# openjamoses/TOSEM-2021-Replication

Measured on NVIDIA H100. Metric: source MB/s scanned (tokenise + line-hash + classify + aggregate), higher is better.
Workload: dtype u8

## Files before the change

tosem-2021-replication_b200/csrc/tsm_scan_walk.cuh:

```cuda
#pragma once
#include "tsm_scan_kernels.cuh"

namespace tsm {

#ifndef TSM_SCAN2_WARPS
#define TSM_SCAN2_WARPS 11
#endif
#ifndef TSM_SCAN2_CTAS
#define TSM_SCAN2_CTAS 2
#endif
#ifndef TSM_WALK_UNROLL
#define TSM_WALK_UNROLL 1
#endif
constexpr int SCAN2_WARPS = TSM_SCAN2_WARPS, SCAN2_CTAS_PER_SM = TSM_SCAN2_CTAS, WALK_UNROLL = TSM_WALK_UNROLL;

constexpr uint32_t NWORD = BUF / 8;
constexpr uint32_t O2_ARUN = BUF;
constexpr uint32_t SLOT_TAIL = NWORD;
constexpr uint32_t RW2_PER_STRIPE = 4;
constexpr uint32_t O2_RW = O2_ARUN + ((NWORD + 1) * 4 + 7) / 8 * 8;
constexpr uint32_t O2_WENT = O2_RW + 32 * RW2_PER_STRIPE * 8;
constexpr uint32_t WENT_CAP = NWORD + 8;
constexpr uint32_t LCAP = 512;
constexpr uint32_t O2_LTAB = O2_WENT + WENT_CAP * 2;
constexpr uint32_t O2_BASE = O2_LTAB + (LCAP + 8) * 2;
constexpr uint32_t Q2_CAP = 64;
constexpr uint32_t O2_Q = O2_BASE + 34 * 8;
constexpr uint32_t O2_CTL = O2_Q + Q2_CAP * 2;
constexpr uint32_t WARP_SMEM2 = ((O2_CTL + 16 + 127) / 128) * 128;
#ifndef TSM_PHASE_CLOCKS
#define TSM_PHASE_CLOCKS 0
#endif
enum ScanPhase { PH_WAIT, PH_ZERO, PH_WALK, PH_SCANS, PH_MIXED, PH_RECORDS, PH_FINISH, PH_LONG, PH_FLUSH, PH_N };
#if TSM_PHASE_CLOCKS
__device__ unsigned long long g_scan_phase_clk[PH_N];
#endif
struct PhaseClock {
#if TSM_PHASE_CLOCKS
  uint32_t* tab;
  long long t;
  __device__ __forceinline__ void mark(int ph, int lane) {
    const long long now = clock64();
    if (lane == 0) atomicAdd(tab + ph, (uint32_t)(now - t));
    t = now;
  }
#else
  __device__ __forceinline__ void mark(int, int) {}
#endif
};

constexpr uint32_t O2_T0A = LUT_BYTES;
constexpr uint32_t O2_PHASE = LUT_BYTES + 512;
constexpr uint32_t CTA_BYTES2 = LUT_BYTES + 512 + (TSM_PHASE_CLOCKS ? 128 : 0);
constexpr uint32_t SCAN2_SMEM = CTA_BYTES2 + SCAN2_WARPS * WARP_SMEM2;
constexpr uint32_t O2_LUTB = SCAN2_SMEM;
constexpr uint32_t SCAN2_SMEM_B = SCAN2_SMEM + 1024;
static_assert(O2_RW % 8 == 0 && O2_WENT % 8 == 0 && O2_LTAB % 2 == 0 && O2_BASE % 8 == 0 && O2_Q % 4 == 0 && O2_CTL % 8 == 0, "alignment");
static_assert(SCAN2_CTAS_PER_SM * (SCAN2_SMEM_B + 1024) <= 233472, "shared memory per SM (228 KB, 1 KB reserved per CTA)");
constexpr uint32_t LR_POS = 0x1FFFu, LR_FIRST = 0x2000u, LR_MIXED = 0x4000u, LR_VIRT = 0x8000u;

constexpr uint32_t B2_FIRST = (1u << 0) | (1u << 6) | (1u << 15), B2_FIN = (1u << 5) | (1u << 14) | (1u << 18);
constexpr uint32_t REVB_BIT = 1u;

struct LutRef { uint32_t four, base; };
__device__ __forceinline__ LutRef lut_ref() { return LutRef{scan_lut()[256 + 12], scan_lut()[256 + 13]}; }
template <bool REVB>
__device__ __forceinline__ void lut_at(uint32_t idx, LutRef t, uint32_t& v, uint32_t& v2) {
  uint32_t addr;
  asm("mad.lo.u32 %0, %1, %2, %3;" : "=r"(addr) : "r"(idx), "r"(t.four), "r"(t.base));
  asm("ld.shared.u32 %0, [%1];" : "=r"(v) : "r"(addr));
  if (REVB) asm("ld.shared.u32 %0, [%1+%2];" : "=r"(v2) : "r"(addr), "n"(O2_LUTB));
}

struct Auto { uint32_t D, D2; };

template <bool REVB>
__device__ __forceinline__ uint32_t step1(Auto& a, uint32_t byte, LutRef t) {
  uint32_t m, m2 = 0;
  lut_at<REVB>(byte, t, m, m2);
  a.D = ((a.D + a.D) | B_FIRST) & m;
  if (!REVB) return a.D;
  a.D2 = ((a.D2 + a.D2) | B2_FIRST) & m2;
  return (a.D & ~REVB_BIT) | ((a.D2 & B2_FIN) ? REVB_BIT : 0u);
}

template <bool REVB>
__device__ __forceinline__ void step8b(unsigned long long w, Auto& a, uint32_t& A, LutRef t) {
  const uint32_t lo = (uint32_t)w, hi = (uint32_t)(w >> 32);
  uint32_t A2 = 0;
#pragma unroll
  for (int k = 0; k < 8; ++k) {
    uint32_t m, m2 = 0;
    lut_at<REVB>(__byte_perm(k < 4 ? lo : hi, 0, 0x4440 + (k & 3)), t, m, m2);
    a.D = ((a.D + a.D) | B_FIRST) & m;
    A |= a.D;
    if (REVB) { a.D2 = ((a.D2 + a.D2) | B2_FIRST) & m2; A2 |= a.D2; }
  }
  if (REVB) A = (A & ~REVB_BIT) | ((A2 & B2_FIN) ? REVB_BIT : 0u);
}

__device__ __forceinline__ uint32_t nl8_of(unsigned long long w) {
  return nl_word((uint32_t)w) | (nl_word((uint32_t)(w >> 32)) << 4);
}
__device__ __forceinline__ unsigned long long low_mask(uint32_t b) {
  return b >= 8u ? ~0ull : ((1ull << (8u * b)) - 1ull);
}
__device__ __forceinline__ unsigned long long ror3_61(unsigned long long r) { return (r >> 3) + ((r & 7ull) << 58); }

struct WalkOut { uint32_t nlw, tail; };

template <bool REVB>
__device__ __noinline__ WalkOut walk2(uint8_t* wb, uint32_t fin, int lane) {
  const uint32_t pos0 = (uint32_t)lane * STRIPE;
  const uint8_t* sp = wb + pos0;
  uint32_t* ar = reinterpret_cast<uint32_t*>(wb + O2_ARUN) + (uint32_t)lane * 17u;
  unsigned long long* rw = reinterpret_cast<unsigned long long*>(wb + O2_RW) + (uint32_t)lane * RW2_PER_STRIPE;
  const LutRef t = lut_ref();
  Auto au{0u, 0u};
  if (lane) {
    uint32_t A = 0;
    step8b<REVB>(*reinterpret_cast<const unsigned long long*>(sp - 8), au, A, t);
  }
  unsigned long long R = 0;
  uint32_t run = 0, nlr = 0;
  auto word = [&](uint32_t k) {
    const unsigned long long w = *reinterpret_cast<const unsigned long long*>(sp + 8u * k);
    uint32_t A = 0;
    step8b<REVB>(w, au, A, t);
    R = ror3_61(R) + fold61(w);
    ar[k] = run;
    nlr = __funnelshift_l(A, nlr, 1);
    const bool nl = (int32_t)A < 0;
    if (nl && (A & fin)) {
      const uint32_t slot = atomicAdd(reinterpret_cast<uint32_t*>(wb + O2_CTL), 1u);
      if (slot < Q2_CAP) reinterpret_cast<uint16_t*>(wb + O2_Q)[slot] = (uint16_t)((uint32_t)lane * 17u + k);
    }
    run = nl ? 0u : (run | A);
  };
#pragma unroll 1
  for (uint32_t g = 0; g < 4; ++g) {
#pragma unroll WALK_UNROLL
    for (uint32_t k = 0; k < 4; ++k) word(4u * g + k);
    rw[g] = R;
  }
  word(16);
  unsigned long long incl = rotl61(canon61(R), (3u * (17u * (uint32_t)lane + 16u)) % 61u);
#pragma unroll
  for (int d = 1; d < 32; d <<= 1) {
    const unsigned long long t = __shfl_up_sync(0xffffffffu, incl, d);
    if (lane >= d) incl = fold61(incl + t);
  }
  unsigned long long excl = __shfl_up_sync(0xffffffffu, incl, 1);
  if (lane == 0) excl = 0;
  unsigned long long* sbase = reinterpret_cast<unsigned long long*>(wb + O2_BASE);
  sbase[lane] = excl;
  if (lane == 31) sbase[32] = incl;
  return WalkOut{__brev(nlr) >> 15, run};
}

template <bool REVB>
__device__ __noinline__ void resolve_mixed(uint8_t* wb, uint32_t g, uint32_t i, uint32_t n_went) {
  const LutRef t = lut_ref();
  Auto au{0u, 0u};
  uint32_t A = 0;
  step8b<REVB>(*reinterpret_cast<const unsigned long long*>(wb + 8u * g - 8u), au, A, t);
  unsigned long long w = *reinterpret_cast<const unsigned long long*>(wb + 8u * g);
  uint32_t pre = 0, post = 0, seen = 0;
#pragma unroll
  for (int b = 0; b < 8; ++b) {
    const uint32_t d = step1<REVB>(au, (uint32_t)w & 0xFFu, t);
    const uint32_t m = (uint32_t)((int32_t)au.D >> 31);
    pre |= d & ~seen;
    seen |= m;
    post = (post | d) & ~m;
    w >>= 8;
  }
  uint32_t* arun = reinterpret_cast<uint32_t*>(wb + O2_ARUN);
  const uint16_t* went = reinterpret_cast<const uint16_t*>(wb + O2_WENT);
  atomicOr(arun + g, pre);
  const uint32_t tgt = i + 1u < n_went ? ((uint32_t)went[i + 1u] & 0x3FFu) : SLOT_TAIL;
  atomicOr(arun + tgt, post);
}

__device__ __forceinline__ void emit_header(const ScanParams& p, uint32_t f, uint32_t line_off, uint32_t len, uint32_t fl) {
  const uint32_t slot = atomicAdd(&p.ctrl->n_hev, 1u);
  if (slot < p.hev_cap) p.hev[slot] = tsm_header_event{f, line_off, len, (fl >> 2) & 1u};
  else p.ctrl->overflow = 1;
}

template <typename Bytes>
__device__ __noinline__ bool starts_with8(Bytes lb, uint32_t s, uint32_t e, unsigned long long pat, uint32_t n, bool need_ws) {
  uint32_t r;
  while (s + 8 <= e && (r = lb.spaces8(s)) != 0) { s += r; if (r < 8) break; }
  while (s < e && is_w(lb(s))) ++s;
  if (s + n + (need_ws ? 1u : 0u) > e) return false;
  const unsigned long long v = lb.load8(s);
  if ((v & low_mask(n)) != pat) return false;
  if (need_ws) {
    const uint32_t c = (uint32_t)(v >> (8u * n)) & 0xFFu;
    if (c != 0x20 && c != 0x09) return false;
    for (uint32_t q = s + n + 1; q < e; ++q)
      if (!is_w(lb(q))) return true;
    return false;
  }
  return true;
}

template <bool REVB, typename Bytes>
__device__ __forceinline__ uint32_t line_flags2(uint32_t s, uint32_t e, uint32_t A, uint32_t g1, uint32_t g2, int ext, Bytes lb, Accum& ac) {
  if (ext == 0) return 0;
  uint32_t fl = (A & (AF_ASSERT | AF_EXPECT | (REVB ? REVB_BIT : 0u))) ? LF_CAND : 0;
  bool hdr;
  if (ext == TSM_EXT_PY) {
    hdr = (A & g1) != 0;
    if (!hdr && (A & g2)) hdr = starts_with8(lb, s, e, 0x7373616C63ull, 5, true);
  } else {
    hdr = (A & g1) != 0 && (A & g2) != 0;
  }
  if (hdr) { fl |= LF_HDR; if ((A & B_F) && starts_with8(lb, s, e, 0x465F54534554ull, 6, false)) fl |= LF_FIX; }
  ac.asserts += fl & LF_CAND;
  ac.hdrs += (fl >> 1) & 1u;
  ac.fixes += (fl >> 2) & 1u;
  return fl;
}

struct FinishState {
  Accum ac;
  uint32_t prev_last;
  unsigned long long prevP;
  uint32_t lh_base, lh_done;
};

template <bool REVB>
__device__ __noinline__ FinishState finish_lines2(const ScanParams& p, uint8_t* wb, const uint32_t* lc, uint32_t n, uint32_t lim,
                                                  bool skip_first, uint32_t f, uint32_t cb, int ext, int lane, FinishState fs) {
  uint16_t* ltab = reinterpret_cast<uint16_t*>(wb + O2_LTAB);
  const uint32_t* arun = reinterpret_cast<const uint32_t*>(wb + O2_ARUN);
  const unsigned long long* t0a = reinterpret_cast<const unsigned long long*>(scan_lut()) + O2_T0A / 8;
  const uint32_t g1 = lc[1], g2 = lc[2];
  const SmemByte lb{wb};
  const bool want_hev = (p.flags & TSM_SCAN_HEADER_EVENTS) != 0, want_lh = (p.flags & TSM_SCAN_LINE_HASHES) != 0;
  Accum a = fs.ac;
  uint32_t nc = 0, lh_done = fs.lh_done;
  uint32_t prev_last = fs.prev_last;
  unsigned long long prevP = fs.prevP;
  for (uint32_t base = 0; base < n; base += 32) {
    const uint32_t j = base + (uint32_t)lane;
    const bool valid = j < n;
    const uint32_t rec = valid ? (uint32_t)ltab[j] : 0u;
    const uint32_t e = rec & LR_POS;
    const bool isv = (rec & LR_VIRT) != 0;
    const uint32_t g = min(e >> 3, NWORD - 1u), b1 = e - 8u * g + (isv ? 0u : 1u);
    const uint32_t l = g / 17u, i = g - 17u * l, c0 = i >> 2, ns = i & 3u;
    unsigned long long R = 0;
    if (c0) R = *reinterpret_cast<const unsigned long long*>(wb + O2_RW + 8u * (l * RW2_PER_STRIPE + c0 - 1u));
    const unsigned long long* wp = reinterpret_cast<const unsigned long long*>(wb) + (g - ns);
#pragma unroll
    for (uint32_t t = 0; t < 3u; ++t)
      if (ns > t) R = ror3_61(R) + fold61(wp[t]);
    const unsigned long long w = *reinterpret_cast<const unsigned long long*>(wb + 8u * g);
    const uint32_t r3g = (3u * g) % 61u;
    const unsigned long long X = ror3_61(R) + fold61(w & low_mask(b1));
    unsigned long long Pn = *reinterpret_cast<const unsigned long long*>(wb + O2_BASE + 8u * l) + rotl61(fold61(fold61(X)), r3g);
    uint32_t r8e = r3g + 8u * (e & 7u);
    if (r8e >= 61u) r8e -= 61u;
    const unsigned long long Pe = isv ? Pn : Pn + M61 - t0a[r8e];
    uint32_t s = __shfl_up_sync(0xffffffffu, e, 1) + 1u;
    unsigned long long Ps = __shfl_up_sync(0xffffffffu, Pn, 1);
    if (lane == 0) { s = prev_last + 1u; Ps = prevP; }
    const int src = base + 32u <= n ? 31 : (int)(n - 1u - base);
    prev_last = __shfl_sync(0xffffffffu, e, src);
    prevP = __shfl_sync(0xffffffffu, Pn, src);
    const bool owned = valid && s < lim && !(s == PRE && skip_first);
    uint32_t fl = 0;
    unsigned long long lh = 0;
    if (owned) {
      const unsigned long long hr = canon61(Pe + 4ull * M61 - Ps);
      const uint32_t sh = (8u * s) % 61u;
      unsigned long long h = rotl61(hr, sh ? 61u - sh : 0u);
      uint32_t len = e - s;
      if (len && lb(e - 1u) == 0x0D) {
        --len;
        const unsigned long long cr = rotl61(0x0Dull, (8u * len) % 61u);
        h = h >= cr ? h - cr : h + M61 - cr;
      }
      a.lines++;
      lh = mix_hash(h, len);
      a.digest += lh;
      uint32_t A = 0;
      if (rec & LR_FIRST) A = arun[isv ? SLOT_TAIL : g];
      else if (rec & LR_MIXED) {
        Auto au{0u, 0u};
        const LutRef t = lut_ref();
        for (uint32_t q = s; q < e; ++q) A |= step1<REVB>(au, lb(q), t);
      }
      fl = line_flags2<REVB>(s, e, A, g1, g2, ext, lb, a);
      if (want_hev && (fl & LF_HDR)) emit_header(p, f, cb + s - PRE, e - s, fl);
    }
    if (want_lh) {
      const uint32_t mo = __ballot_sync(0xffffffffu, owned);
      const uint32_t slot = fs.lh_base + lh_done + __popc(mo & ((1u << lane) - 1u));
      if (owned && slot < p.lh_cap) {
        p.lh_hash[slot] = lh;
        p.lh_end[slot] = cb + e - PRE;
        p.lh_flag[slot] = (uint8_t)(fl & LF_CAND);
      }
      lh_done += __popc(mo);
    }
    __syncwarp();
    const uint32_t mc = __ballot_sync(0xffffffffu, fl & LF_CAND);
    if (fl & LF_CAND) ltab[nc + __popc(mc & ((1u << lane) - 1u))] = (uint16_t)s;
    nc += __popc(mc);
  }
  __syncwarp();
  if (nc && p.cand_cap) {
    const uint32_t cbase = warp_reserve(&p.ctrl->n_cand, nc, lane);
    for (uint32_t i = (uint32_t)lane; i < nc; i += 32) {
      const uint32_t slot = cbase + i;
      if (slot < p.cand_cap) p.cand[slot] = ((unsigned long long)f << 32) | (cb + (uint32_t)ltab[i] - PRE);
      else p.ctrl->overflow = 1;
    }
  }
  __syncwarp();
  fs.ac = a;
  fs.prev_last = prev_last;
  fs.prevP = prevP;
  fs.lh_done = lh_done;
  return fs;
}

template <bool REVB>
__device__ __noinline__ Accum long_line(const ScanParams& p, const uint32_t* lc, uint32_t f, uint32_t size, int ext,
                                        uint32_t s, uint32_t lh_slot, Accum ac) {
  const HbmByte lb{p.arena + (uint32_t)p.off[f]};
  uint32_t e = s;
  while (e < size && lb(e) != '\n') ++e;
  const uint32_t k0 = s >> 3, k1 = (e - 1u) >> 3;
  const LutRef t = lut_ref();
  Auto au{0u, 0u};
  uint32_t A = 0;
  unsigned long long R = 0;
#pragma unroll 1
  for (uint32_t k = k0; k <= k1; ++k) {
    unsigned long long w = __ldg(reinterpret_cast<const unsigned long long*>(lb.b) + k);
    if (k == k0) w &= ~0ull << (8u * (s & 7u));
    if (k == k1) w &= low_mask(e - 8u * k);
    uint32_t Aw = 0;
    step8b<REVB>(w, au, Aw, t);
    A |= Aw;
    R = ror3_61(R) + fold61(w);
  }
  unsigned long long h = rotl61(canon61(R), (3u * (k1 - k0) + 61u * 8u - 8u * (s & 7u)) % 61u);
  uint32_t len = e - s;
  if (lb(e - 1u) == 0x0D) {
    --len;
    const unsigned long long cr = rotl61(0x0Dull, (8u * len) % 61u);
    h = h >= cr ? h - cr : h + M61 - cr;
  }
  const unsigned long long lh = mix_hash(h, len);
  ac.lines++;
  ac.digest += lh;
  const uint32_t fl = line_flags2<REVB>(s, e, A, lc[1], lc[2], ext, lb, ac);
  if ((fl & LF_CAND) && p.cand_cap) {
    const uint32_t slot = atomicAdd(&p.ctrl->n_cand, 1u);
    if (slot < p.cand_cap) p.cand[slot] = ((unsigned long long)f << 32) | s;
    else p.ctrl->overflow = 1;
  }
  if ((fl & LF_HDR) && (p.flags & TSM_SCAN_HEADER_EVENTS)) emit_header(p, f, s, e - s, fl);
  if ((p.flags & TSM_SCAN_LINE_HASHES) && lh_slot < p.lh_cap) {
    p.lh_hash[lh_slot] = lh;
    p.lh_end[lh_slot] = e;
    p.lh_flag[lh_slot] = (uint8_t)(fl & LF_CAND);
  }
  return ac;
}

template <bool REVB>
__device__ __forceinline__ void process_chunk2(const ScanParams& p, const uint32_t* lc, uint8_t* wb, uint32_t uslot, uint32_t f,
                                               uint32_t cb, uint32_t size, int ext, int lane, PhaseClock& pc) {
  const uint32_t ce = min(cb + CH, size);
  const uint32_t le = min(ce + EXT, size);
  const uint32_t lim = PRE + (ce - cb);
  const uint32_t lim2 = PRE + (le - cb);
  const bool skip_first = (cb != 0) && (wb[PRE - 1] != '\n');
  __syncwarp();
  if (lane < 2) reinterpret_cast<unsigned long long*>(wb)[lane] = 0ull;
  {
    const uint32_t za = (lim2 + 7u) & ~7u;
    if ((uint32_t)lane < za - lim2) wb[lim2 + lane] = 0;
    for (uint32_t q = za + 8u * (uint32_t)lane; q < BUF; q += 256u) *reinterpret_cast<unsigned long long*>(wb + q) = 0ull;
  }
  if (lane == 0) *reinterpret_cast<uint32_t*>(wb + O2_CTL) = 0u;
  __syncwarp();
  pc.mark(PH_ZERO, lane);
  const WalkOut wo = walk2<REVB>(wb, lc[0], lane);
  pc.mark(PH_WALK, lane);
  const uint32_t w0 = 17u * (uint32_t)lane, lim_w = (lim + 7u) >> 3;
  const uint32_t ownbits = lim_w <= w0 ? 0u : (lim_w - w0 >= 17u ? 0x1FFFFu : (1u << (lim_w - w0)) - 1u);
  const uint32_t extbits = wo.nlw & ~ownbits;
  const uint32_t gx = __reduce_min_sync(0xffffffffu, extbits ? w0 + (uint32_t)__ffs((int)extbits) - 1u : 0xFFFFu);
  uint32_t kept = wo.nlw & ownbits;
  if (gx - w0 < 17u) kept |= 1u << (gx - w0);
  uint32_t tv = wo.tail, tf = wo.nlw != 0u;
  const uint32_t cnt = __popc(kept);
  uint32_t incl = cnt;
#pragma unroll
  for (int d = 1; d < 32; d <<= 1) {
    const uint32_t uv = __shfl_up_sync(0xffffffffu, tv, d), uf = __shfl_up_sync(0xffffffffu, tf, d);
    const uint32_t t = __shfl_up_sync(0xffffffffu, incl, d);
    if (lane >= d) { if (!tf) tv |= uv; tf |= uf; incl += t; }
  }
  uint32_t carry = __shfl_up_sync(0xffffffffu, tv, 1);
  if (lane == 0) carry = 0;
  const uint32_t tail_all = __shfl_sync(0xffffffffu, tv, 31);
  const uint32_t n_went = __shfl_sync(0xffffffffu, incl, 31), ebase = incl - cnt;
  uint16_t* went = reinterpret_cast<uint16_t*>(wb + O2_WENT);
  uint32_t* arun = reinterpret_cast<uint32_t*>(wb + O2_ARUN);
  {
    uint32_t b = kept, idx = ebase;
    while (b) { went[idx++] = (uint16_t)(w0 + (uint32_t)__ffs((int)b) - 1u); b &= b - 1u; }
    if (wo.nlw) arun[w0 + (uint32_t)__ffs((int)wo.nlw) - 1u] |= carry;
    if (lane == 0) arun[SLOT_TAIL] = tail_all;
  }
  __syncwarp();
  pc.mark(PH_SCANS, lane);
  {
    const uint32_t nq_all = *reinterpret_cast<const uint32_t*>(wb + O2_CTL);
    const uint16_t* q = reinterpret_cast<const uint16_t*>(wb + O2_Q);
    if (nq_all <= Q2_CAP) {
      for (uint32_t base = 0; base < nq_all; base += 32) {
        const uint32_t t = base + (uint32_t)lane;
        const uint32_t g = t < nq_all ? (uint32_t)q[t] : 0u;
        const uint32_t l = g / 17u, k = g - 17u * l;
        const uint32_t m = __shfl_sync(0xffffffffu, kept, (int)l), eb = __shfl_sync(0xffffffffu, ebase, (int)l);
        const bool act = t < nq_all && ((m >> k) & 1u);
        const uint32_t i = eb + __popc(m & ((1u << k) - 1u));
        if (act) resolve_mixed<REVB>(wb, g, i, n_went);
        __syncwarp();
        if (act) went[i] |= 0x8000u;
        __syncwarp();
      }
    } else if (lc[0]) {
      for (uint32_t base = 0; base < n_went; base += 32) {
        const uint32_t i = base + (uint32_t)lane;
        if (i < n_went) resolve_mixed<REVB>(wb, (uint32_t)went[i] & 0x3FFu, i, n_went);
        __syncwarp();
        if (i < n_went) went[i] |= 0x8000u;
        __syncwarp();
      }
    }
  }
  pc.mark(PH_MIXED, lane);
  uint16_t* ltab = reinterpret_cast<uint16_t*>(wb + O2_LTAB);
  FinishState fs{{0, 0, 0, 0, 0}, PRE - 1u, 0ull, 0u, 0u};
  const bool want_lh = (p.flags & TSM_SCAN_LINE_HASHES) != 0;
  if (want_lh) {
    uint32_t tot = 0;
    for (uint32_t j = (uint32_t)lane; j < n_went; j += 32)
      tot += __popc(nl8_of(*reinterpret_cast<const unsigned long long*>(wb + 8u * ((uint32_t)went[j] & 0x3FFu))));
    tot = __reduce_add_sync(0xffffffffu, tot) + 1u;
    uint32_t base = 0;
    if (lane == 0) {
      base = atomicAdd(&p.ctrl->n_lh, tot);
      if (base + tot > p.lh_cap) p.ctrl->lh_overflow = 1;
      p.unit_out[uslot] = base;
    }
    fs.lh_base = __shfl_sync(0xffffffffu, base, 0);
  }
  uint32_t n_rec = 0, last_nl = PRE - 1u;
  for (uint32_t base = 0; base < n_went; base += 32) {
    const uint32_t j = base + (uint32_t)lane;
    const uint32_t ge = j < n_went ? (uint32_t)went[j] : 0u;
    const uint32_t g = ge & 0x3FFu;
    uint32_t m = j < n_went ? nl8_of(*reinterpret_cast<const unsigned long long*>(wb + 8u * g)) : 0u;
    const uint32_t c = __popc(m);
    uint32_t in2 = c;
#pragma unroll
    for (int d = 1; d < 32; d <<= 1) {
      const uint32_t t = __shfl_up_sync(0xffffffffu, in2, d);
      if (lane >= d) in2 += t;
    }
    if (base + 32u >= n_went) {
      const uint32_t lastl = n_went - 1u - base;
      last_nl = __shfl_sync(0xffffffffu, 8u * g + 31u - (uint32_t)__clz((int)(m | 1u)), (int)lastl);
    }
    uint32_t off = n_rec + in2 - c;
    uint32_t rec = 8u * g + LR_FIRST + ((ge >> 15) << 14);
    while (m) {
      ltab[off++] = (uint16_t)(rec + (uint32_t)__ffs((int)m) - 1u);
      rec &= ~LR_FIRST;
      m &= m - 1u;
    }
    n_rec += __shfl_sync(0xffffffffu, in2, 31);
    __syncwarp();
    if (n_rec + 256u > LCAP && base + 32u < n_went) {
      pc.mark(PH_RECORDS, lane);
      fs = finish_lines2<REVB>(p, wb, lc, n_rec, lim, skip_first, f, cb, ext, lane, fs);
      pc.mark(PH_FINISH, lane);
      n_rec = 0;
    }
  }
  const uint32_t tail_start = last_nl + 1u;
  bool tail_long = false;
  if (tail_start < lim && !(skip_first && n_went == 0u)) {
    if (le == size) {
      if (tail_start < lim2) { if (lane == 0) ltab[n_rec] = (uint16_t)(lim2 | LR_VIRT | LR_FIRST); ++n_rec; }
    } else tail_long = true;
  }
  __syncwarp();
  pc.mark(PH_RECORDS, lane);
  if (n_rec) fs = finish_lines2<REVB>(p, wb, lc, n_rec, lim, skip_first, f, cb, ext, lane, fs);
  pc.mark(PH_FINISH, lane);
  Accum ac = fs.ac;
  if (tail_long && lane == 0) ac = long_line<REVB>(p, lc, f, size, ext, cb + tail_start - PRE, fs.lh_base + fs.lh_done, ac);
  pc.mark(PH_LONG, lane);
  ac.lines = __reduce_add_sync(0xffffffffu, ac.lines);
  ac.asserts = __reduce_add_sync(0xffffffffu, ac.asserts);
  ac.hdrs = __reduce_add_sync(0xffffffffu, ac.hdrs);
  ac.fixes = __reduce_add_sync(0xffffffffu, ac.fixes);
  {
    const uint32_t dlo = (uint32_t)ac.digest, dhi = (uint32_t)(ac.digest >> 32);
    const unsigned long long s0 = __reduce_add_sync(0xffffffffu, dlo & 0xFFFFu);
    const unsigned long long s1 = __reduce_add_sync(0xffffffffu, dlo >> 16);
    const unsigned long long s2 = __reduce_add_sync(0xffffffffu, dhi);
    ac.digest = s0 + (s1 << 16) + (s2 << 32);
  }
  if (want_lh && lane == 0) p.unit_lines[uslot] = ac.lines;
  if (lane == 0) {
    tsm_file_stat* st = p.stats + f;
    if (size <= CH) {
      *st = tsm_file_stat{ac.lines, ac.asserts, ac.hdrs, ac.fixes, ac.digest};
    } else {
      if (ac.lines) atomicAdd(&st->n_lines, ac.lines);
      if (ac.asserts) atomicAdd(&st->n_assert, ac.asserts);
      if (ac.hdrs) atomicAdd(&st->n_headers, ac.hdrs);
      if (ac.fixes) atomicAdd(&st->n_fixture, ac.fixes);
      if (ac.digest) atomicAdd(reinterpret_cast<unsigned long long*>(&st->digest), ac.digest);
    }
  }
  pc.mark(PH_FLUSH, lane);
}

template <bool REVB>
__global__ void __launch_bounds__(SCAN2_WARPS * 32, SCAN2_CTAS_PER_SM) k_scan_t(const __grid_constant__ ScanParams p) {
  extern __shared__ __align__(128) uint8_t smem[];
  uint32_t* lut_all = reinterpret_cast<uint32_t*>(smem);
  for (int i = threadIdx.x; i < 256; i += blockDim.x) lut_all[i] = c_lut[i];
  if (threadIdx.x < 12) {
    const int t = threadIdx.x, lang = t >> 2, q = t & 3;
    const uint32_t g1 = lang == 0 ? PY_G1 : CJ_G1, g2 = lang == 0 ? PY_G2 : CJ_G2;
    const uint32_t v = q == 0 ? (AF_ASSERT | AF_EXPECT | g1 | g2 | B_F | (REVB ? REVB_BIT : 0u)) : (q == 1 ? g1 : (q == 2 ? g2 : 0u));
    lut_all[256 + t] = lang == 2 ? 0u : v;
  }
  if (threadIdx.x == 12) lut_all[256 + 12] = p.four;
  if (threadIdx.x == 13) lut_all[256 + 13] = smem_u32(lut_all);
  if (REVB) for (int i = threadIdx.x; i < 256; i += blockDim.x) lut_all[O2_LUTB / 4 + i] = c_lut_b[i];
  PhaseClock pc;
#if TSM_PHASE_CLOCKS
  pc.tab = reinterpret_cast<uint32_t*>(smem + O2_PHASE);
  if (threadIdx.x < PH_N) pc.tab[threadIdx.x] = 0u;
#endif
  if (threadIdx.x >= 32 && threadIdx.x < 32 + 61)
    reinterpret_cast<unsigned long long*>(smem + O2_T0A)[threadIdx.x - 32] = rotl61(0x0Aull, threadIdx.x - 32);
  __syncthreads();
  const int warp = threadIdx.x >> 5, lane = threadIdx.x & 31;
  uint8_t* wb = smem + CTA_BYTES2 + warp * WARP_SMEM2;
  uint64_t* bar = reinterpret_cast<uint64_t*>(wb + O2_CTL + 8);
  uint32_t* phase = reinterpret_cast<uint32_t*>(wb + O2_CTL + 4);
  if (lane == 0) { mbar_init(bar, 1); fence_mbar_init(); *phase = 0u; }
  __syncwarp();
  const uint32_t n_units = p.slab->n_units;
  Unit cur = claim_unit(p, n_units, lane);
#if TSM_PHASE_CLOCKS
  pc.t = clock64();
#endif
  while (cur.u < n_units) {
    fence_proxy_async();
    __syncwarp();
    if (lane == 0) issue_load(p, wb, bar, cur.fo, cur.size, cur.cb);
    const Unit nxt = claim_unit(p, n_units, lane);
    const uint32_t ph = *phase;
    while (!mbar_try_wait(bar, ph)) {}
    __syncwarp();
    if (lane == 0) *phase = ph ^ 1u;
    pc.mark(PH_WAIT, lane);
    const uint32_t lang = cur.ext == 0 ? 2u : (cur.ext == TSM_EXT_PY ? 0u : 1u);
    process_chunk2<REVB>(p, lut_all + 256u + 4u * lang, wb, p.unit_base + cur.u, cur.f, cur.cb, cur.size, cur.ext, lane, pc);
    __syncwarp();
    cur = nxt;
  }
#if TSM_PHASE_CLOCKS
  __syncthreads();
  if (threadIdx.x < PH_N) atomicAdd(&g_scan_phase_clk[threadIdx.x], (unsigned long long)pc.tab[threadIdx.x]);
#endif
}

template __global__ void k_scan_t<false>(const __grid_constant__ ScanParams);
template __global__ void k_scan_t<true>(const __grid_constant__ ScanParams);

}
```

Measured before the change: 616,900.

## Hash lines from end-inclusive prefix and subtract newline constant algebraically

Each line hash now uses the prefix value that includes the terminating byte at each line end (Pe) rather than a separate pre-newline prefix. A constant-shift correction for the preceding newline is subtracted after the rotation, which removes the per-CTA shared-memory rotation table and its per-line lookup. The warp shuffles are merged so the carry from the last lane comes from one indexed shuffle, the prefix-fold loop is made branch-free, and header and fix counters are incremented inside the branch. This cuts shared-memory loads and shuffles per line, but correctness depends on the modular identity holding for virtual line ends and for the initial carry value.

Result: no change. 618,500 (median of 6 runs) (+0.3%).

```diff
diff --git a/tosem-2021-replication_b200/csrc/tsm_scan_walk.cuh b/tosem-2021-replication_b200/csrc/tsm_scan_walk.cuh
--- a/tosem-2021-replication_b200/csrc/tsm_scan_walk.cuh
+++ b/tosem-2021-replication_b200/csrc/tsm_scan_walk.cuh
@@ -49,9 +49,8 @@
 #endif
 };
 
-constexpr uint32_t O2_T0A = LUT_BYTES;
-constexpr uint32_t O2_PHASE = LUT_BYTES + 512;
-constexpr uint32_t CTA_BYTES2 = LUT_BYTES + 512 + (TSM_PHASE_CLOCKS ? 128 : 0);
+constexpr uint32_t O2_PHASE = LUT_BYTES;
+constexpr uint32_t CTA_BYTES2 = LUT_BYTES + (TSM_PHASE_CLOCKS ? 128 : 0);
 constexpr uint32_t SCAN2_SMEM = CTA_BYTES2 + SCAN2_WARPS * WARP_SMEM2;
 constexpr uint32_t O2_LUTB = SCAN2_SMEM;
 constexpr uint32_t SCAN2_SMEM_B = SCAN2_SMEM + 1024;
@@ -217,17 +216,21 @@
   } else {
     hdr = (A & g1) != 0 && (A & g2) != 0;
   }
-  if (hdr) { fl |= LF_HDR; if ((A & B_F) && starts_with8(lb, s, e, 0x465F54534554ull, 6, false)) fl |= LF_FIX; }
+  if (hdr) {
+    fl |= LF_HDR;
+    ac.hdrs++;
+    if ((A & B_F) && starts_with8(lb, s, e, 0x465F54534554ull, 6, false)) { fl |= LF_FIX; ac.fixes++; }
+  }
   ac.asserts += fl & LF_CAND;
-  ac.hdrs += (fl >> 1) & 1u;
-  ac.fixes += (fl >> 2) & 1u;
   return fl;
 }
+
+constexpr unsigned long long NL_BEFORE = 0x0Aull << 53;
 
 struct FinishState {
   Accum ac;
   uint32_t prev_last;
-  unsigned long long prevP;
+  unsigned long long prevPe;
   uint32_t lh_base, lh_done;
 };
 
@@ -236,41 +239,42 @@
                                                   bool skip_first, uint32_t f, uint32_t cb, int ext, int lane, FinishState fs) {
   uint16_t* ltab = reinterpret_cast<uint16_t*>(wb + O2_LTAB);
   const uint32_t* arun = reinterpret_cast<const uint32_t*>(wb + O2_ARUN);
-  const unsigned long long* t0a = reinterpret_cast<const unsigned long long*>(scan_lut()) + O2_T0A / 8;
   const uint32_t g1 = lc[1], g2 = lc[2];
   const SmemByte lb{wb};
   const bool want_hev = (p.flags & TSM_SCAN_HEADER_EVENTS) != 0, want_lh = (p.flags & TSM_SCAN_LINE_HASHES) != 0;
   Accum a = fs.ac;
   uint32_t nc = 0, lh_done = fs.lh_done;
   uint32_t prev_last = fs.prev_last;
-  unsigned long long prevP = fs.prevP;
+  unsigned long long prevPe = fs.prevPe;
   for (uint32_t base = 0; base < n; base += 32) {
     const uint32_t j = base + (uint32_t)lane;
     const bool valid = j < n;
     const uint32_t rec = valid ? (uint32_t)ltab[j] : 0u;
     const uint32_t e = rec & LR_POS;
     const bool isv = (rec & LR_VIRT) != 0;
-    const uint32_t g = min(e >> 3, NWORD - 1u), b1 = e - 8u * g + (isv ? 0u : 1u);
+    const uint32_t g = min(e >> 3, NWORD - 1u), b1 = e - 8u * g;
     const uint32_t l = g / 17u, i = g - 17u * l, c0 = i >> 2, ns = i & 3u;
     unsigned long long R = 0;
     if (c0) R = *reinterpret_cast<const unsigned long long*>(wb + O2_RW + 8u * (l * RW2_PER_STRIPE + c0 - 1u));
     const unsigned long long* wp = reinterpret_cast<const unsigned long long*>(wb) + (g - ns);
 #pragma unroll
-    for (uint32_t t = 0; t < 3u; ++t)
-      if (ns > t) R = ror3_61(R) + fold61(wp[t]);
+    for (uint32_t t = 0; t < 3u; ++t) {
+      const unsigned long long Rt = ror3_61(R) + fold61(wp[t]);
+      R = ns > t ? Rt : R;
+    }
     const unsigned long long w = *reinterpret_cast<const unsigned long long*>(wb + 8u * g);
-    const uint32_t r3g = (3u * g) % 61u;
     const unsigned long long X = ror3_61(R) + fold61(w & low_mask(b1));
-    unsigned long long Pn = *reinterpret_cast<const unsigned long long*>(wb + O2_BASE + 8u * l) + rotl61(fold61(fold61(X)), r3g);
-    uint32_t r8e = r3g + 8u * (e & 7u);
-    if (r8e >= 61u) r8e -= 61u;
-    const unsigned long long Pe = isv ? Pn : Pn + M61 - t0a[r8e];
-    uint32_t s = __shfl_up_sync(0xffffffffu, e, 1) + 1u;
-    unsigned long long Ps = __shfl_up_sync(0xffffffffu, Pn, 1);
-    if (lane == 0) { s = prev_last + 1u; Ps = prevP; }
+    const unsigned long long Pe = *reinterpret_cast<const unsigned long long*>(wb + O2_BASE + 8u * l) + rotl61(fold61(fold61(X)), (3u * g) % 61u);
     const int src = base + 32u <= n ? 31 : (int)(n - 1u - base);
-    prev_last = __shfl_sync(0xffffffffu, e, src);
-    prevP = __shfl_sync(0xffffffffu, Pn, src);
+    const int from = lane ? lane - 1 : src;
+    uint32_t s = __shfl_sync(0xffffffffu, e, from) + 1u;
+    unsigned long long Ps = __shfl_sync(0xffffffffu, Pe, from);
+    if (lane == 0) {
+      const uint32_t e_last = s - 1u;
+      const unsigned long long P_last = Ps;
+      s = prev_last + 1u; Ps = prevPe;
+      prev_last = e_last; prevPe = P_last;
+    }
     const bool owned = valid && s < lim && !(s == PRE && skip_first);
     uint32_t fl = 0;
     unsigned long long lh = 0;
@@ -278,6 +282,7 @@
       const unsigned long long hr = canon61(Pe + 4ull * M61 - Ps);
       const uint32_t sh = (8u * s) % 61u;
       unsigned long long h = rotl61(hr, sh ? 61u - sh : 0u);
+      h = h >= NL_BEFORE ? h - NL_BEFORE : h + M61 - NL_BEFORE;
       uint32_t len = e - s;
       if (len && lb(e - 1u) == 0x0D) {
         --len;
@@ -324,7 +329,7 @@
   __syncwarp();
   fs.ac = a;
   fs.prev_last = prev_last;
-  fs.prevP = prevP;
+  fs.prevPe = prevPe;
   fs.lh_done = lh_done;
   return fs;
 }
@@ -452,7 +457,7 @@
   }
   pc.mark(PH_MIXED, lane);
   uint16_t* ltab = reinterpret_cast<uint16_t*>(wb + O2_LTAB);
-  FinishState fs{{0, 0, 0, 0, 0}, PRE - 1u, 0ull, 0u, 0u};
+  FinishState fs{{0, 0, 0, 0, 0}, PRE - 1u, M61 - rotl61(0x0Aull, (8u * (PRE - 1u)) % 61u), 0u, 0u};
   const bool want_lh = (p.flags & TSM_SCAN_LINE_HASHES) != 0;
   if (want_lh) {
     uint32_t tot = 0;
@@ -560,8 +565,6 @@
   pc.tab = reinterpret_cast<uint32_t*>(smem + O2_PHASE);
   if (threadIdx.x < PH_N) pc.tab[threadIdx.x] = 0u;
 #endif
-  if (threadIdx.x >= 32 && threadIdx.x < 32 + 61)
-    reinterpret_cast<unsigned long long*>(smem + O2_T0A)[threadIdx.x - 32] = rotl61(0x0Aull, threadIdx.x - 32);
   __syncthreads();
   const int warp = threadIdx.x >> 5, lane = threadIdx.x & 31;
   uint8_t* wb = smem + CTA_BYTES2 + warp * WARP_SMEM2;
```
